# YBZh/Point-DAE

Hardware: AMD Instinct MI355X
Metric: pretrain point-clouds/sec (N=1024,G=64) (higher is better)
Workload: dtype f32 (3xbf16 exact-split operands, fp32 accumulate); 1 GPU; cfg3/cfg4: pretrain_PointCAE_transformer_dropout_patch_affine_r3_maskpatch_p0005_whole.yaml full train step (fwd+loss+bwd+AdamW); local_batch=128, global_batch=128, npoints=1024, num_group=64, group_size=32, parallelism=dp1, launch=hipGraph replay, reductions=float atomics, grad_allreduce=none (1 rank)

## Files before the change

### point_dae_amd/csrc/block.hip

```cpp
#include "common.h"

namespace pdae {

__device__ __forceinline__ float wave_sum(float v) {
#pragma unroll
  for (int o = 32; o >= 1; o >>= 1) v += __shfl_xor(v, o, kWave);
  return v;
}

constexpr int LN_MAX4 = 8;

__global__ __launch_bounds__(256) void add_layernorm_fwd_kernel(
    int M, int C, const float* __restrict__ x, const float* __restrict__ pos,
    const float* __restrict__ gamma, const float* __restrict__ beta, float eps,
    float* __restrict__ xsum, float* __restrict__ y, float* __restrict__ mean,
    float* __restrict__ rstd, const float* __restrict__ br, const float* __restrict__ bias,
    const float* __restrict__ keep, int T, int br_slabs) {
  const int row = blockIdx.x * 4 + (threadIdx.x >> 6);
  if (row >= M) return;
  const int lane = lane_id();
  const int n4 = C >> 2;
  const float k = keep ? keep[row / T] : 1.f;
  float4 v[LN_MAX4];
  float s = 0.f;
#pragma unroll
  for (int i = 0; i < LN_MAX4; ++i) {
    const int c4 = lane + i * kWave;
    if (c4 < n4) {
      float4 a = *reinterpret_cast<const float4*>(x + (size_t)row * C + c4 * 4);
      if (br) {
        float4 t = *reinterpret_cast<const float4*>(br + (size_t)row * C + c4 * 4);
        for (int q = 1; q < br_slabs; ++q) {
          const float4 u = *reinterpret_cast<const float4*>(br + ((size_t)q * M + row) * C + c4 * 4);
          t.x += u.x, t.y += u.y, t.z += u.z, t.w += u.w;
        }
        if (bias) {
          const float4 b = *reinterpret_cast<const float4*>(bias + c4 * 4);
          t.x += b.x, t.y += b.y, t.z += b.z, t.w += b.w;
        }
        if (keep) t.x *= k, t.y *= k, t.z *= k, t.w *= k;
        a.x += t.x, a.y += t.y, a.z += t.z, a.w += t.w;
      }
      if (pos) {
        const float4 p = *reinterpret_cast<const float4*>(pos + (size_t)row * C + c4 * 4);
        a.x += p.x, a.y += p.y, a.z += p.z, a.w += p.w;
      }
      if (pos || br) store_wt4(xsum + (size_t)row * C + c4 * 4, a);
      v[i] = a;
      s += (a.x + a.y) + (a.z + a.w);
    }
  }
  const float mu = wave_sum(s) / (float)C;
  float q = 0.f;
#pragma unroll
  for (int i = 0; i < LN_MAX4; ++i) {
    const int c4 = lane + i * kWave;
    if (c4 < n4) {
      const float dx = v[i].x - mu, dy = v[i].y - mu, dz = v[i].z - mu, dw = v[i].w - mu;
      q += (dx * dx + dy * dy) + (dz * dz + dw * dw);
    }
  }
  const float rs = rsqrtf(wave_sum(q) / (float)C + eps);
  if (lane == 0) {
    mean[row] = mu;
    rstd[row] = rs;
  }
#pragma unroll
  for (int i = 0; i < LN_MAX4; ++i) {
    const int c4 = lane + i * kWave;
    if (c4 < n4) {
      const float4 g = *reinterpret_cast<const float4*>(gamma + c4 * 4);
      const float4 b = *reinterpret_cast<const float4*>(beta + c4 * 4);
      float4 o;
      o.x = (v[i].x - mu) * rs * g.x + b.x;
      o.y = (v[i].y - mu) * rs * g.y + b.y;
      o.z = (v[i].z - mu) * rs * g.z + b.z;
      o.w = (v[i].w - mu) * rs * g.w + b.w;
      store_wt4(y + (size_t)row * C + c4 * 4, o);
    }
  }
}

template <int NS, int NW>
__global__ __launch_bounds__(NW * 64) void layernorm_bwd_kernel(
    int M, int C, int rows, const float* __restrict__ dy, const float* __restrict__ x,
    const float* __restrict__ mean, const float* __restrict__ rstd,
    const float* __restrict__ gamma, const float* __restrict__ dres, float* __restrict__ dx,
    float* __restrict__ dgamma, float* __restrict__ dbeta, const float* __restrict__ keep, int T,
    float* __restrict__ da, float* __restrict__ dbias, int dy_slabs, float* __restrict__ dacc, int dacc_mode,
    float* __restrict__ part) {
  extern __shared__ float red[];
  const int lane = lane_id(), w = threadIdx.x >> 6;
  const int n4 = C >> 2;
  const float4 zero4 = make_float4(0.f, 0.f, 0.f, 0.f);
  float4 ag[NS], ab[NS], g[NS], ac[NS];
#pragma unroll
  for (int i = 0; i < NS; ++i) {
    ag[i] = ab[i] = ac[i] = zero4;
    const int c4 = lane + i * kWave;
    g[i] = c4 < n4 ? *reinterpret_cast<const float4*>(gamma + c4 * 4) : zero4;
  }
  float4 d[NS], xv[NS], e[NS];
  float mu = 0.f, rs = 0.f, kp = 1.f;
  auto load_row = [&](int row) {
#pragma unroll
    for (int i = 0; i < NS; ++i) {
      const int c4 = lane + i * kWave;
      const bool on = c4 < n4 && row < M;
      const size_t off = (size_t)row * C + c4 * 4;
      d[i] = on ? *reinterpret_cast<const float4*>(dy + off) : zero4;
      for (int q = 1; q < dy_slabs; ++q) {
        const float4 u = on ? *reinterpret_cast<const float4*>(dy + (size_t)q * M * C + off) : zero4;
        d[i].x += u.x, d[i].y += u.y, d[i].z += u.z, d[i].w += u.w;
      }
      xv[i] = on ? *reinterpret_cast<const float4*>(x + off) : zero4;
      e[i] = (on && dres) ? *reinterpret_cast<const float4*>(dres + off) : zero4;
    }
    mu = row < M ? mean[row] : 0.f;
    rs = row < M ? rstd[row] : 0.f;
    kp = (keep && row < M) ? keep[row / T] : 1.f;
  };
  const int row0 = blockIdx.x * rows + w;
  load_row(row0);
  for (int rr = 0; rr < rows / NW; ++rr) {
    const int row = row0 + rr * NW;
    if (row >= M) break;
    float4 gd[NS], xh[NS];
    float s1 = 0.f, s2 = 0.f;
    const float rs_ = rs, kp_ = kp;
#pragma unroll
    for (int i = 0; i < NS; ++i) {
      xh[i] = make_float4((xv[i].x - mu) * rs, (xv[i].y - mu) * rs, (xv[i].z - mu) * rs, (xv[i].w - mu) * rs);
      gd[i] = make_float4(d[i].x * g[i].x, d[i].y * g[i].y, d[i].z * g[i].z, d[i].w * g[i].w);
      s1 += (gd[i].x + gd[i].y) + (gd[i].z + gd[i].w);
      s2 += (gd[i].x * xh[i].x + gd[i].y * xh[i].y) + (gd[i].z * xh[i].z + gd[i].w * xh[i].w);
      ag[i].x += d[i].x * xh[i].x, ag[i].y += d[i].y * xh[i].y, ag[i].z += d[i].z * xh[i].z, ag[i].w += d[i].w * xh[i].w;
      ab[i].x += d[i].x, ab[i].y += d[i].y, ab[i].z += d[i].z, ab[i].w += d[i].w;
    }
    float4 sk[NS];
#pragma unroll
    for (int i = 0; i < NS; ++i) sk[i] = e[i];
    if (rr + 1 < rows / NW) load_row(row + NW);
    const float m1 = wave_sum(s1) / (float)C, m2 = wave_sum(s2) / (float)C;
#pragma unroll
    for (int i = 0; i < NS; ++i) {
      const int c4 = lane + i * kWave;
      if (c4 < n4) {
        float4 o;
        o.x = rs_ * (gd[i].x - m1 - xh[i].x * m2) + sk[i].x;
        o.y = rs_ * (gd[i].y - m1 - xh[i].y * m2) + sk[i].y;
        o.z = rs_ * (gd[i].z - m1 - xh[i].z * m2) + sk[i].z;
        o.w = rs_ * (gd[i].w - m1 - xh[i].w * m2) + sk[i].w;
        store_wt4(dx + (size_t)row * C + c4 * 4, o);
        if (dacc_mode == 1) {
          store_wt4(dacc + (size_t)row * C + c4 * 4, o);
        } else if (dacc_mode == 2) {
          float4 t = *reinterpret_cast<const float4*>(dacc + (size_t)row * C + c4 * 4);
          t.x += o.x, t.y += o.y, t.z += o.z, t.w += o.w;
          *reinterpret_cast<float4*>(dacc + (size_t)row * C + c4 * 4) = t;
        }
        if (dbias) {
          if (keep) o.x *= kp_, o.y *= kp_, o.z *= kp_, o.w *= kp_;
          if (da) store_wt4(da + (size_t)row * C + c4 * 4, o);
          ac[i].x += o.x, ac[i].y += o.y, ac[i].z += o.z, ac[i].w += o.w;
        }
      }
    }
  }
  const int nred = dbias ? 3 : 2;
  float* mine = red + (size_t)w * nred * C;
#pragma unroll
  for (int i = 0; i < NS; ++i) {
    const int c4 = lane + i * kWave;
    if (c4 < n4) {
      *reinterpret_cast<float4*>(mine + c4 * 4) = ag[i];
      *reinterpret_cast<float4*>(mine + C + c4 * 4) = ab[i];
      if (dbias) *reinterpret_cast<float4*>(mine + 2 * C + c4 * 4) = ac[i];
    }
  }
  __syncthreads();
  for (int c = threadIdx.x; c < nred * C; c += NW * 64) {
    float t = 0.f;
#pragma unroll 4
    for (int k = 0; k < NW; ++k) t += red[(size_t)k * nred * C + c];
    col_add(c < C ? dgamma + c : (c < 2 * C ? dbeta + (c - C) : dbias + (c - 2 * C)), part, blockIdx.x,
            nred * C, c, t);
  }
}

__global__ __launch_bounds__(256) void bias_gelu_fwd_kernel(long long n4, int C4,
                                                            const float4* __restrict__ z,
                                                            const float4* __restrict__ bias,
                                                            float4* __restrict__ h) {
  const long long i = (long long)blockIdx.x * 256 + threadIdx.x;
  if (i >= n4) return;
  const float4 v = z[i], b = bias[i % C4];
  h[i] = make_float4(gelu_f(v.x + b.x), gelu_f(v.y + b.y), gelu_f(v.z + b.z), gelu_f(v.w + b.w));
}

constexpr int CS_NW = 16, CS_ROWS = 4 * CS_NW;
__device__ __forceinline__ void colsum_finish(float4 s, float4 (*part)[64], float* __restrict__ out, int c,
                                              int N, float* __restrict__ det) {
  const int lane = threadIdx.x & 63, w = threadIdx.x >> 6;
  part[w][lane] = s;
  __syncthreads();
  if (w == 0 && c < N && out) {
    float4 t = part[0][lane];
#pragma unroll
    for (int k = 1; k < CS_NW; ++k) {
      const float4 u = part[k][lane];
      t.x += u.x, t.y += u.y, t.z += u.z, t.w += u.w;
    }
    if (det) {
      *reinterpret_cast<float4*>(det + (size_t)blockIdx.y * N + c) = t;
    } else {
      atomicAdd(out + c + 0, t.x), atomicAdd(out + c + 1, t.y);
      atomicAdd(out + c + 2, t.z), atomicAdd(out + c + 3, t.w);
    }
  }
}

__global__ __launch_bounds__(CS_NW * 64) void bias_gelu_bwd_kernel(int M, int C, const float* __restrict__ z,
                                                            const float* __restrict__ bias,
                                                            const float* __restrict__ dh,
                                                            float* __restrict__ dz,
                                                            float* __restrict__ dbias,
                                                            int rows_per_split, float* __restrict__ det) {
  __shared__ float4 part[CS_NW][64];
  const int lane = threadIdx.x & 63, w = threadIdx.x >> 6;
  const int c = (blockIdx.x * 64 + lane) * 4;
  const int mbeg = blockIdx.y * rows_per_split, mend = min(M, mbeg + rows_per_split);
  float4 s = make_float4(0.f, 0.f, 0.f, 0.f);
  if (c < C) {
    const float4 b = *reinterpret_cast<const float4*>(bias + c);
#pragma unroll 4
    for (int m = mbeg + w; m < mend; m += CS_NW) {
      const float4 v = *reinterpret_cast<const float4*>(z + (size_t)m * C + c);
      const float4 d = *reinterpret_cast<const float4*>(dh + (size_t)m * C + c);
      float4 o;
      o.x = d.x * gelu_grad_f(v.x + b.x);
      o.y = d.y * gelu_grad_f(v.y + b.y);
      o.z = d.z * gelu_grad_f(v.z + b.z);
      o.w = d.w * gelu_grad_f(v.w + b.w);
      *reinterpret_cast<float4*>(dz + (size_t)m * C + c) = o;
      s.x += o.x, s.y += o.y, s.z += o.z, s.w += o.w;
    }
  }
  colsum_finish(s, part, dbias, c, C, det);
}

__global__ __launch_bounds__(256) void gelu_fwd_kernel(long long n4, const float4* __restrict__ z,
                                                       float4* __restrict__ h) {
  const long long i = (long long)blockIdx.x * 256 + threadIdx.x;
  if (i >= n4) return;
  const float4 v = z[i];
  h[i] = make_float4(gelu_f(v.x), gelu_f(v.y), gelu_f(v.z), gelu_f(v.w));
}

__global__ __launch_bounds__(256) void gelu_bwd_kernel(long long n4, const float4* __restrict__ z,
                                                       const float4* __restrict__ dh,
                                                       float4* __restrict__ dz) {
  const long long i = (long long)blockIdx.x * 256 + threadIdx.x;
  if (i >= n4) return;
  const float4 v = z[i], d = dh[i];
  dz[i] = make_float4(d.x * gelu_grad_f(v.x), d.y * gelu_grad_f(v.y), d.z * gelu_grad_f(v.z),
                      d.w * gelu_grad_f(v.w));
}

__global__ __launch_bounds__(256) void scale_residual_kernel(long long n4, int C4, int T,
                                                             const float4* __restrict__ a,
                                                             const float4* __restrict__ bias,
                                                             const float* __restrict__ keep,
                                                             const float4* __restrict__ res,
                                                             float4* __restrict__ y) {
  const long long i = (long long)blockIdx.x * 256 + threadIdx.x;
  if (i >= n4) return;
  const long long row = i / C4;
  float4 v = a[i];
  if (bias) {
    const float4 b = bias[i - row * C4];
    v.x += b.x, v.y += b.y, v.z += b.z, v.w += b.w;
  }
  if (keep) {
    const float k = keep[row / T];
    v.x *= k, v.y *= k, v.z *= k, v.w *= k;
  }
  if (res) {
    const float4 r = res[i];
    v.x += r.x, v.y += r.y, v.z += r.z, v.w += r.w;
  }
  y[i] = v;
}

template <int LPR>
__global__ __launch_bounds__(CS_NW * 64) void colsum2_kernel(int M, int N, const float* __restrict__ X,
                                                             float* __restrict__ out, int rows_per_split,
                                                             float* __restrict__ det) {
  __shared__ float4 part[CS_NW][64];
  constexpr int RPW = 64 / LPR;
  const int lane = threadIdx.x & 63, w = threadIdx.x >> 6;
  const int c = (blockIdx.x * 64 + (lane % LPR)) * 4;
  const int mbeg = blockIdx.y * rows_per_split, mend = min(M, mbeg + rows_per_split);
  float4 s = make_float4(0.f, 0.f, 0.f, 0.f);
  if (c < N) {
#pragma unroll 4
    for (int m = mbeg + w * RPW + lane / LPR; m < mend; m += CS_NW * RPW) {
      const float4 v = *reinterpret_cast<const float4*>(X + (size_t)m * N + c);
      s.x += v.x, s.y += v.y, s.z += v.z, s.w += v.w;
    }
  }
  if (LPR < 64) {
#pragma unroll
    for (int o = 32; o >= LPR; o >>= 1) {
      s.x += __shfl_xor(s.x, o, kWave), s.y += __shfl_xor(s.y, o, kWave);
      s.z += __shfl_xor(s.z, o, kWave), s.w += __shfl_xor(s.w, o, kWave);
    }
    if (lane >= LPR) s = make_float4(0.f, 0.f, 0.f, 0.f), part[w][lane] = s;
  }
  colsum_finish(s, part, (LPR < 64 && lane >= LPR) ? nullptr : out, c, N, det);
}

__global__ __launch_bounds__(CS_NW * 64) void scale_colsum_kernel(int M, int N, int T,
                                                                  const float* __restrict__ X,
                                                                  const float* __restrict__ keep,
                                                                  float* __restrict__ Y, float* __restrict__ out,
                                                                  int rows_per_split, float* __restrict__ det) {
  __shared__ float4 part[CS_NW][64];
  const int lane = threadIdx.x & 63, w = threadIdx.x >> 6;
  const int c = (blockIdx.x * 64 + lane) * 4;
  const int mbeg = blockIdx.y * rows_per_split, mend = min(M, mbeg + rows_per_split);
  float4 s = make_float4(0.f, 0.f, 0.f, 0.f);
  if (c < N) {
#pragma unroll 4
    for (int m = mbeg + w; m < mend; m += CS_NW) {
      float4 v = *reinterpret_cast<const float4*>(X + (size_t)m * N + c);
      const float k = keep[m / T];
      v.x *= k, v.y *= k, v.z *= k, v.w *= k;
      *reinterpret_cast<float4*>(Y + (size_t)m * N + c) = v;
      s.x += v.x, s.y += v.y, s.z += v.z, s.w += v.w;
    }
  }
  colsum_finish(s, part, out, c, N, det);
}

}

using namespace pdae;

static int cs_rows(int M) {
  int rows = CS_ROWS;
  if ((M + rows - 1) / rows > 256) rows = CS_NW * ((M + 256 * CS_NW - 1) / (256 * CS_NW));
  return rows;
}

static int ln_forward(const char* what, int M, int C, int T, const float* x, const float* br,
                      const float* bias, const float* keep, const float* pos, const float* gamma,
                      const float* beta, float eps, float* xsum, float* y, float* mean, float* rstd,
                      int br_slabs, pdae_stream_t stream) {
  if (M < 0 || C <= 0 || C % 4 != 0 || C > 4 * kWave * LN_MAX4 || T <= 0 || br_slabs < 1 || br_slabs > 8)
    return bad_arg("layernorm forward: C must be a multiple of 4, at most 2048; T > 0; 1..8 slabs");
  if (M == 0) return PDAE_OK;
  if (!x || !gamma || !beta || !y || !mean || !rstd || ((pos || br) && !xsum) || ((bias || keep) && !br))
    return bad_arg("layernorm forward: null pointer");
  hipLaunchKernelGGL(add_layernorm_fwd_kernel, dim3((M + 3) / 4), dim3(256), 0, as_stream(stream), M,
                     C, x, pos, gamma, beta, eps, xsum, y, mean, rstd, br, bias, keep, T, br_slabs);
  return check_launch(what);
}

extern "C" int pdae_add_layernorm_forward(int M, int C, const float* x, const float* pos,
                                          const float* gamma, const float* beta, float eps,
                                          float* xsum, float* y, float* mean, float* rstd,
                                          pdae_stream_t stream) {
  return ln_forward("add_layernorm_forward", M, C, 1, x, nullptr, nullptr, nullptr, pos, gamma, beta, eps,
                    xsum, y, mean, rstd, 1, stream);
}

extern "C" int pdae_residual_layernorm_forward(int M, int C, int T, const float* a, int a_slabs, const float* bias,
                                               const float* keep, const float* res, const float* pos,
                                               const float* gamma, const float* beta, float eps,
                                               float* xsum, float* y, float* mean, float* rstd,
                                               pdae_stream_t stream) {
  if (!a) return bad_arg("residual_layernorm_forward: null pointer");
  return ln_forward("residual_layernorm_forward", M, C, T, res, a, bias, keep, pos, gamma, beta, eps, xsum,
                    y, mean, rstd, a_slabs, stream);
}

static int ln_backward(const char* what, int M, int C, int T, const float* dy, int dy_slabs, const float* x,
                       const float* mean, const float* rstd, const float* gamma, const float* dres,
                       const float* keep, float* dx, float* da, float* dgamma, float* dbeta, float* dbias,
                       int accumulate, float* dacc, int dacc_mode, pdae_stream_t stream) {
  if (dacc_mode < 0 || dacc_mode > 2 || (dacc_mode && !dacc)) return bad_arg("layernorm backward: bad dacc");
  if (M < 0 || C <= 0 || C % 4 != 0 || C > 4 * kWave * LN_MAX4 || T <= 0 || dy_slabs < 1 || dy_slabs > 8)
    return bad_arg("layernorm backward: C must be a multiple of 4, at most 2048; T > 0; 1..8 slabs");
  if (!dgamma || !dbeta) return bad_arg("layernorm backward: null pointer");
  hipStream_t s = as_stream(stream);
  if (!accumulate) {
    (void)hipMemsetAsync(dgamma, 0, sizeof(float) * C, s);
    (void)hipMemsetAsync(dbeta, 0, sizeof(float) * C, s);
    if (dbias) (void)hipMemsetAsync(dbias, 0, sizeof(float) * C, s);
  }
  if (M == 0) return check_launch(what);
  if (!dy || !x || !mean || !rstd || !gamma || !dx || ((keep || da) && !dbias) || (keep && !da))
    return bad_arg("layernorm backward: null pointer");
  const int nred = dbias ? 3 : 2;
  int rows, blocks;
  if (C <= 512) {
    rows = 16 * (M >= 6144 ? 2 : 1);
  } else {
    rows = 4 * ((M + 4 * 256 - 1) / (4 * 256));
    if (rows > 32) rows = 32;
  }
  blocks = (M + rows - 1) / rows;
  int rc = PDAE_OK;
  float* part = static_cast<float*>(det_workspace(sizeof(float) * (size_t)blocks * nred * C, &rc));
  if (rc) return rc;
  bool parked = false;
  if (!part && (part = deferred_take(blocks, nred * C, dgamma, C, dbeta, C, dbias, dbias ? C : 0))) parked = true;
  if (C <= 512)
    hipLaunchKernelGGL((layernorm_bwd_kernel<2, 16>), dim3(blocks), dim3(1024), 16 * nred * C * sizeof(float), s, M,
                       C, rows, dy, x, mean, rstd, gamma, dres, dx, dgamma, dbeta, keep, T, da, dbias, dy_slabs,
                       dacc, dacc_mode, part);
  else
    hipLaunchKernelGGL((layernorm_bwd_kernel<LN_MAX4, 4>), dim3(blocks), dim3(256), 4 * nred * C * sizeof(float), s,
                       M, C, rows, dy, x, mean, rstd, gamma, dres, dx, dgamma, dbeta, keep, T, da, dbias, dy_slabs,
                       dacc, dacc_mode, part);
  if (part && !parked) return det_reduce(s, blocks, nred * C, part, dgamma, C, dbeta, C, dbias, dbias ? C : 0);
  return check_launch(what);
}

extern "C" int pdae_layernorm_backward(int M, int C, const float* dy, int dy_slabs, const float* x,
                                       const float* mean, const float* rstd, const float* gamma,
                                       const float* dres, float* dx, float* dgamma, float* dbeta,
                                       int accumulate, float* dacc, int dacc_mode, pdae_stream_t stream) {
  return ln_backward("layernorm_backward", M, C, 1, dy, dy_slabs, x, mean, rstd, gamma, dres, nullptr, dx, nullptr,
                     dgamma, dbeta, nullptr, accumulate, dacc, dacc_mode, stream);
}

extern "C" int pdae_residual_layernorm_backward(int M, int C, int T, const float* dy, int dy_slabs, const float* x,
                                                const float* mean, const float* rstd,
                                                const float* gamma, const float* dres,
                                                const float* keep, float* dx, float* da, float* dgamma,
                                                float* dbeta, float* dbias, int accumulate,
                                                float* dacc, int dacc_mode, pdae_stream_t stream) {
  if (!dbias) return bad_arg("residual_layernorm_backward: null pointer");
  return ln_backward("residual_layernorm_backward", M, C, T, dy, dy_slabs, x, mean, rstd, gamma, dres, keep, dx, da,
                     dgamma, dbeta, dbias, accumulate, dacc, dacc_mode, stream);
}

extern "C" int pdae_gelu_forward(long long n, const float* z, float* h, pdae_stream_t stream) {
  if (n < 0 || n % 4 != 0) return bad_arg("gelu_forward: n must be a multiple of 4");
  if (n == 0) return PDAE_OK;
  if (!z || !h) return bad_arg("gelu_forward: null pointer");
  hipLaunchKernelGGL(gelu_fwd_kernel, dim3((unsigned)((n / 4 + 255) / 256)), dim3(256), 0,
                     as_stream(stream), n / 4, reinterpret_cast<const float4*>(z),
                     reinterpret_cast<float4*>(h));
  return check_launch("gelu_forward");
}

extern "C" int pdae_gelu_backward(long long n, const float* z, const float* dh, float* dz,
                                  pdae_stream_t stream) {
  if (n < 0 || n % 4 != 0) return bad_arg("gelu_backward: n must be a multiple of 4");
  if (n == 0) return PDAE_OK;
  if (!z || !dh || !dz) return bad_arg("gelu_backward: null pointer");
  hipLaunchKernelGGL(gelu_bwd_kernel, dim3((unsigned)((n / 4 + 255) / 256)), dim3(256), 0,
                     as_stream(stream), n / 4, reinterpret_cast<const float4*>(z),
                     reinterpret_cast<const float4*>(dh), reinterpret_cast<float4*>(dz));
  return check_launch("gelu_backward");
}

extern "C" int pdae_bias_gelu_forward(int M, int C, const float* z, const float* bias, float* h,
                                      pdae_stream_t stream) {
  if (M < 0 || C <= 0 || C % 4 != 0) return bad_arg("bias_gelu_forward: C must be a positive multiple of 4");
  if (M == 0) return PDAE_OK;
  if (!z || !bias || !h) return bad_arg("bias_gelu_forward: null pointer");
  const long long n4 = (long long)M * (C / 4);
  hipLaunchKernelGGL(bias_gelu_fwd_kernel, dim3((unsigned)((n4 + 255) / 256)), dim3(256), 0,
                     as_stream(stream), n4, C / 4, reinterpret_cast<const float4*>(z),
                     reinterpret_cast<const float4*>(bias), reinterpret_cast<float4*>(h));
  return check_launch("bias_gelu_forward");
}

extern "C" int pdae_bias_gelu_backward(int M, int C, const float* z, const float* bias,
                                       const float* dh, float* dz, float* dbias, int accumulate,
                                       pdae_stream_t stream) {
  if (M < 0 || C <= 0 || C % 4 != 0) return bad_arg("bias_gelu_backward: C must be a positive multiple of 4");
  if (!dbias) return bad_arg("bias_gelu_backward: null pointer");
  hipStream_t s = as_stream(stream);
  if (!accumulate) (void)hipMemsetAsync(dbias, 0, sizeof(float) * (size_t)C, s);
  if (M == 0) return check_launch("bias_gelu_backward");
  if (!z || !bias || !dh || !dz) return bad_arg("bias_gelu_backward: null pointer");
  const int rows = cs_rows(M), P = (M + rows - 1) / rows;
  int rc = PDAE_OK;
  float* det = static_cast<float*>(det_workspace(sizeof(float) * (size_t)P * C, &rc));
  if (rc) return rc;
  hipLaunchKernelGGL(bias_gelu_bwd_kernel, dim3((C + 255) / 256, P), dim3(CS_NW * 64), 0, s, M, C, z, bias, dh, dz,
                     dbias, rows, det);
  if (det) return det_reduce(s, P, C, det, dbias, C);
  return check_launch("bias_gelu_backward");
}

extern "C" int pdae_scale_residual(int M, int C, int T, const float* a, const float* bias,
                                   const float* keep, const float* res, float* y,
                                   pdae_stream_t stream) {
  if (M < 0 || C <= 0 || C % 4 != 0 || T <= 0) return bad_arg("scale_residual: bad size");
  if (M == 0) return PDAE_OK;
  if (!a || !y) return bad_arg("scale_residual: null pointer");
  const long long n4 = (long long)M * (C / 4);
  hipLaunchKernelGGL(scale_residual_kernel, dim3((unsigned)((n4 + 255) / 256)), dim3(256), 0,
                     as_stream(stream), n4, C / 4, T, reinterpret_cast<const float4*>(a),
                     reinterpret_cast<const float4*>(bias), keep, reinterpret_cast<const float4*>(res),
                     reinterpret_cast<float4*>(y));
  return check_launch("scale_residual");
}

extern "C" int pdae_colsum(int M, int N, const float* X, float* out, int accumulate,
                           pdae_stream_t stream) {
  if (M < 0 || N <= 0 || N % 4 != 0) return bad_arg("colsum: N must be a positive multiple of 4");
  if (!out) return bad_arg("colsum: null pointer");
  hipStream_t s = as_stream(stream);
  if (!accumulate) (void)hipMemsetAsync(out, 0, sizeof(float) * (size_t)N, s);
  if (M == 0) return check_launch("colsum");
  if (!X) return bad_arg("colsum: null pointer");
  const int rows = cs_rows(M), P = (M + rows - 1) / rows;
  int rc = PDAE_OK;
  float* det = static_cast<float*>(det_workspace(sizeof(float) * (size_t)P * N, &rc));
  if (rc) return rc;
  if (N == 128)
    hipLaunchKernelGGL(colsum2_kernel<32>, dim3(1, P), dim3(CS_NW * 64), 0, s, M, N, X, out, rows, det);
  else if (N == 64)
    hipLaunchKernelGGL(colsum2_kernel<16>, dim3(1, P), dim3(CS_NW * 64), 0, s, M, N, X, out, rows, det);
  else
    hipLaunchKernelGGL(colsum2_kernel<64>, dim3((N + 255) / 256, P), dim3(CS_NW * 64), 0, s, M, N, X, out, rows, det);
  if (det) return det_reduce(s, P, N, det, out, N);
  return check_launch("colsum");
}

extern "C" int pdae_scale_colsum(int M, int N, int T, const float* X, const float* keep, float* Y,
                                 float* out, int accumulate, pdae_stream_t stream) {
  if (M < 0 || N <= 0 || N % 4 != 0 || T <= 0) return bad_arg("scale_colsum: N must be a positive multiple of 4, T > 0");
  hipStream_t s = as_stream(stream);
  if (out && !accumulate) (void)hipMemsetAsync(out, 0, sizeof(float) * (size_t)N, s);
  if (M == 0) return check_launch("scale_colsum");
  if (!X || !keep || !Y) return bad_arg("scale_colsum: null pointer");
  const int rows = cs_rows(M), P = (M + rows - 1) / rows;
  int rc = PDAE_OK;
  float* det = out ? static_cast<float*>(det_workspace(sizeof(float) * (size_t)P * N, &rc)) : nullptr;
  if (rc) return rc;
  hipLaunchKernelGGL(scale_colsum_kernel, dim3((N + 255) / 256, P), dim3(CS_NW * 64), 0, s, M, N, T, X, keep, Y,
                     out, rows, det);
  if (det) return det_reduce(s, P, N, det, out, N);
  return check_launch("scale_colsum");
}


namespace pdae {

__global__ __launch_bounds__(256) void drop_path_keep_kernel(int n, int B, const float* __restrict__ r,
                                                             const float* __restrict__ keep, float* __restrict__ out) {
  const int i = blockIdx.x * 256 + threadIdx.x;
  if (i >= n) return;
  const float k = keep[i / B];
  out[i] = floorf(r[i] + k) / k;
}

__global__ __launch_bounds__(256) void pos_embed_fc1_kernel(int M, int H, const float* __restrict__ xyz,
                                                            const long long* __restrict__ rows,
                                                            const float* __restrict__ w1, const float* __restrict__ b1,
                                                            float* __restrict__ h, float* __restrict__ gp,
                                                            float* __restrict__ xp) {
  const int q = H / 4;
  const long long i = (long long)blockIdx.x * 256 + threadIdx.x;
  if (i >= (long long)M * q) return;
  const int m = (int)(i / q), c = (int)(i % q) * 4;
  const long long src = rows ? rows[m] : m;
  const float x0 = xyz[src * 3 + 0], x1 = xyz[src * 3 + 1], x2 = xyz[src * 3 + 2];
  if (c == 0) *reinterpret_cast<float4*>(xp + (size_t)m * 4) = make_float4(x0, x1, x2, 0.f);
  float hv[4], gv[4];
#pragma unroll
  for (int e = 0; e < 4; ++e) {
    const float* w = w1 + (size_t)(c + e) * 3;
    const float z = fmaf(x2, w[2], fmaf(x1, w[1], x0 * w[0])) + b1[c + e];
    const float cdf = 0.5f * (1.0f + erff(z * 0.70710678118654752440f));
    const float pdf = 0.39894228040143267794f * expf(-0.5f * z * z);
    hv[e] = z * cdf, gv[e] = cdf + z * pdf;
  }
  *reinterpret_cast<float4*>(h + (size_t)m * H + c) = make_float4(hv[0], hv[1], hv[2], hv[3]);
  *reinterpret_cast<float4*>(gp + (size_t)m * H + c) = make_float4(gv[0], gv[1], gv[2], gv[3]);
}

__global__ __launch_bounds__(256) void tail_rows_gather_kernel(long long n4, int C4, int T, int tail, const float4* __restrict__ a,
                                                               const float4* __restrict__ b, float4* __restrict__ a_t,
                                                               float4* __restrict__ b_t) {
  const long long i = (long long)blockIdx.x * 256 + threadIdx.x;
  if (i >= n4) return;
  const long long row = i / C4;
  const int c = (int)(i - row * C4);
  const long long smp = row / tail;
  const long long src = (smp * T + (T - tail) + (row - smp * tail)) * C4 + c;
  a_t[i] = a[src];
  if (b) b_t[i] = b[src];
}
__global__ __launch_bounds__(256) void tail_rows_scatter_kernel(long long n4, int C4, int T, int tail, const float4* __restrict__ da_t,
                                                                const float4* __restrict__ db_t, float4* __restrict__ da,
                                                                float4* __restrict__ db) {
  const long long i = (long long)blockIdx.x * 256 + threadIdx.x;
  if (i >= n4) return;
  const long long row = i / C4;
  const int c = (int)(i - row * C4);
  const long long smp = row / T;
  const int t = (int)(row - smp * T) - (T - tail);
  const float4 zero = make_float4(0.f, 0.f, 0.f, 0.f);
  const long long src = (smp * tail + t) * C4 + c;
  da[i] = t >= 0 ? da_t[src] : zero;
  if (db) db[i] = t >= 0 ? db_t[src] : zero;
}

__global__ __launch_bounds__(256) void slab_sum_epi_kernel(long long n4, int N4, int S, const float4* __restrict__ slabs,
                                                           const float4* __restrict__ bias, int epi,
                                                           const float4* __restrict__ z, float4* __restrict__ y) {
  const long long i = (long long)blockIdx.x * 256 + threadIdx.x;
  if (i >= n4) return;
  float4 a = slabs[i];
  for (int q = 1; q < S; ++q) {
    const float4 v = slabs[(size_t)q * n4 + i];
    a.x += v.x, a.y += v.y, a.z += v.z, a.w += v.w;
  }
  if (bias) {
    const float4 b = bias[i % N4];
    a.x += b.x, a.y += b.y, a.z += b.z, a.w += b.w;
  }
  if (epi == 1) a.x = a.x > 0.f ? a.x : 0.f, a.y = a.y > 0.f ? a.y : 0.f, a.z = a.z > 0.f ? a.z : 0.f, a.w = a.w > 0.f ? a.w : 0.f;
  if (epi == 4) {
    const float4 m = z[i];
    a.x = m.x > 0.f ? a.x : 0.f, a.y = m.y > 0.f ? a.y : 0.f, a.z = m.z > 0.f ? a.z : 0.f, a.w = m.w > 0.f ? a.w : 0.f;
  }
  y[i] = a;
}

}

static int tail_check(int B, int T, int tail, int C) {
  if (B < 0 || T <= 0 || tail <= 0 || tail > T || C <= 0 || C % 4 != 0) return bad_arg("tail_rows: B >= 0, 0 < tail <= T, C a positive multiple of 4");
  return PDAE_OK;
}
extern "C" int pdae_tail_rows_gather(int B, int T, int tail, int C, const float* a, const float* b, float* a_t, float* b_t,
                                     pdae_stream_t stream) {
  using namespace pdae;
  int rc = tail_check(B, T, tail, C);
  if (rc) return rc;
  if (B == 0) return PDAE_OK;
  if (!a || !a_t || (b && !b_t)) return bad_arg("tail_rows_gather: null pointer");
  const long long n4 = (long long)B * tail * (C / 4);
  hipLaunchKernelGGL(tail_rows_gather_kernel, dim3((unsigned)((n4 + 255) / 256)), dim3(256), 0, as_stream(stream), n4, C / 4, T, tail,
                     reinterpret_cast<const float4*>(a), reinterpret_cast<const float4*>(b), reinterpret_cast<float4*>(a_t),
                     reinterpret_cast<float4*>(b_t));
  return check_launch("tail_rows_gather");
}
extern "C" int pdae_tail_rows_scatter(int B, int T, int tail, int C, const float* da_t, const float* db_t, float* da, float* db,
                                      pdae_stream_t stream) {
  using namespace pdae;
  int rc = tail_check(B, T, tail, C);
  if (rc) return rc;
  if (B == 0) return PDAE_OK;
  if (!da_t || !da || (db && !db_t)) return bad_arg("tail_rows_scatter: null pointer");
  const long long n4 = (long long)B * T * (C / 4);
  hipLaunchKernelGGL(tail_rows_scatter_kernel, dim3((unsigned)((n4 + 255) / 256)), dim3(256), 0, as_stream(stream), n4, C / 4, T, tail,
                     reinterpret_cast<const float4*>(da_t), reinterpret_cast<const float4*>(db_t), reinterpret_cast<float4*>(da),
                     reinterpret_cast<float4*>(db));
  return check_launch("tail_rows_scatter");
}

extern "C" int pdae_slab_sum_epi(int S, int M, int N, const float* slabs, const float* bias, int epi, const float* Z, float* Y,
                                 pdae_stream_t stream) {
  using namespace pdae;
  if (S <= 0 || S > 8 || M < 0 || N <= 0 || N % 4 != 0) return bad_arg("slab_sum_epi: 1..8 slabs, M >= 0, N a positive multiple of 4");
  if (epi != 0 && epi != 1 && epi != 4) return bad_arg("slab_sum_epi: epi 0 (store), 1 (ReLU) or 4 (mask by Z > 0)");
  if (M == 0) return PDAE_OK;
  if (!slabs || !Y || (epi == 4 && !Z)) return bad_arg("slab_sum_epi: null pointer");
  const long long n4 = (long long)M * (N / 4);
  hipLaunchKernelGGL(slab_sum_epi_kernel, dim3((unsigned)((n4 + 255) / 256)), dim3(256), 0, as_stream(stream), n4, N / 4, S,
                     reinterpret_cast<const float4*>(slabs), reinterpret_cast<const float4*>(bias), epi,
                     reinterpret_cast<const float4*>(Z), reinterpret_cast<float4*>(Y));
  return check_launch("slab_sum_epi");
}

extern "C" int pdae_drop_path_keep(int sites, int B, const float* r, const float* keep, float* out, pdae_stream_t stream) {
  using namespace pdae;
  if (sites < 0 || B < 0) return bad_arg("drop_path_keep: negative size");
  if (sites == 0 || B == 0) return PDAE_OK;
  if (!r || !keep || !out) return bad_arg("drop_path_keep: null pointer");
  const int n = sites * B;
  hipLaunchKernelGGL(drop_path_keep_kernel, dim3((n + 255) / 256), dim3(256), 0, as_stream(stream), n, B, r, keep, out);
  return check_launch("drop_path_keep");
}

extern "C" int pdae_pos_embed_fc1(int M, int H, const float* xyz, const int64_t* rows, const float* w1, const float* b1,
                                  float* h, float* gp, float* xp, pdae_stream_t stream) {
  using namespace pdae;
  if (M < 0 || H <= 0 || H % 4 != 0) return bad_arg("pos_embed_fc1: M >= 0, H a positive multiple of 4 required");
  if (M == 0) return PDAE_OK;
  if (!xyz || !w1 || !b1 || !h || !gp || !xp) return bad_arg("pos_embed_fc1: null pointer");
  const long long n = (long long)M * (H / 4);
  hipLaunchKernelGGL(pos_embed_fc1_kernel, dim3((unsigned)((n + 255) / 256)), dim3(256), 0, as_stream(stream), M, H, xyz,
                     reinterpret_cast<const long long*>(rows), w1, b1, h, gp, xp);
  return check_launch("pos_embed_fc1");
}
```

Before: 13230 clouds/s.

## Specialize layernorm kernels by slab count, bias, pos and residual flags

Adds templated forward and backward layernorm kernels, specialized at compile time on column-chunk count, number of summed slabs and whether bias, pos or residual inputs exist. The forward kernel issues all loads up front, and the backward kernel prefetches the next row and the dacc value ahead of the reduction, so memory latency overlaps with compute. The tail scatter kernel now skips its loads for padded rows. An environment variable can fall back to the legacy kernels, and the extra instantiations cost code size and register pressure.

```diff
diff --git a/point_dae_amd/csrc/block.hip b/point_dae_amd/csrc/block.hip
--- a/point_dae_amd/csrc/block.hip
+++ b/point_dae_amd/csrc/block.hip
@@ -1,3 +1,6 @@
+#include <stdlib.h>
+#include <string.h>
+
 #include "common.h"
 
 namespace pdae {
@@ -10,7 +13,7 @@
 
 constexpr int LN_MAX4 = 8;
 
-__global__ __launch_bounds__(256) void add_layernorm_fwd_kernel(
+__global__ __launch_bounds__(256) void add_layernorm_fwd_legacy_kernel(
     int M, int C, const float* __restrict__ x, const float* __restrict__ pos,
     const float* __restrict__ gamma, const float* __restrict__ beta, float eps,
     float* __restrict__ xsum, float* __restrict__ y, float* __restrict__ mean,
@@ -81,8 +84,99 @@
   }
 }
 
+__device__ __forceinline__ float4 ld4(const float* p) { return *reinterpret_cast<const float4*>(p); }
+__device__ __forceinline__ void add4(float4& a, const float4& b) { a.x += b.x, a.y += b.y, a.z += b.z, a.w += b.w; }
+
+template <int NS, int SLABS, bool BIAS, bool POS>
+__global__ __launch_bounds__(256) void add_layernorm_fwd_kernel(
+    int M, int C, const float* __restrict__ x, const float* __restrict__ pos,
+    const float* __restrict__ gamma, const float* __restrict__ beta, float eps,
+    float* __restrict__ xsum, float* __restrict__ y, float* __restrict__ mean,
+    float* __restrict__ rstd, const float* __restrict__ br, const float* __restrict__ bias,
+    const float* __restrict__ keep, int T, int br_slabs) {
+  constexpr bool BR = SLABS != 0;
+  constexpr int SL = SLABS > 0 ? SLABS : 1;
+  const int row = blockIdx.x * 4 + (threadIdx.x >> 6);
+  if (row >= M) return;
+  const int lane = lane_id();
+  const int n4 = C >> 2;
+  const float4 zero4 = make_float4(0.f, 0.f, 0.f, 0.f);
+  float k = 1.f;
+  if (keep) k = keep[row / T];
+  float4 v[NS], u[SL][NS], bb[NS], pp[NS], g[NS], be[NS];
+#pragma unroll
+  for (int i = 0; i < NS; ++i) {
+    v[i] = bb[i] = pp[i] = g[i] = be[i] = zero4;
+#pragma unroll
+    for (int q = 0; q < SL; ++q) u[q][i] = zero4;
+    const int c4 = lane + i * kWave;
+    if (c4 < n4) {
+      const size_t off = (size_t)row * C + c4 * 4;
+      v[i] = ld4(x + off);
+      if (BR) {
+#pragma unroll
+        for (int q = 0; q < SL; ++q) u[q][i] = ld4(br + (size_t)q * M * C + off);
+      }
+      if (POS) pp[i] = ld4(pos + off);
+      if (BR && BIAS) bb[i] = ld4(bias + c4 * 4);
+      g[i] = ld4(gamma + c4 * 4);
+      be[i] = ld4(beta + c4 * 4);
+    }
+  }
+  float s = 0.f;
+#pragma unroll
+  for (int i = 0; i < NS; ++i) {
+    const int c4 = lane + i * kWave;
+    if (c4 < n4) {
+      float4 a = v[i];
+      if (BR) {
+        float4 t = u[0][i];
+#pragma unroll
+        for (int q = 1; q < SL; ++q) add4(t, u[q][i]);
+        if (SLABS < 0) {
+          for (int q = 1; q < br_slabs; ++q) add4(t, ld4(br + ((size_t)q * M + row) * C + c4 * 4));
+        }
+        if (BIAS) add4(t, bb[i]);
+        if (keep) t.x *= k, t.y *= k, t.z *= k, t.w *= k;
+        add4(a, t);
+      }
+      if (POS) add4(a, pp[i]);
+      if (POS || BR) store_wt4(xsum + (size_t)row * C + c4 * 4, a);
+      v[i] = a;
+      s += (a.x + a.y) + (a.z + a.w);
+    }
+  }
+  const float mu = wave_sum(s) / (float)C;
+  float q = 0.f;
+#pragma unroll
+  for (int i = 0; i < NS; ++i) {
+    const int c4 = lane + i * kWave;
+    if (c4 < n4) {
+      const float dx = v[i].x - mu, dy = v[i].y - mu, dz = v[i].z - mu, dw = v[i].w - mu;
+      q += (dx * dx + dy * dy) + (dz * dz + dw * dw);
+    }
+  }
+  const float rs = rsqrtf(wave_sum(q) / (float)C + eps);
+  if (lane == 0) {
+    mean[row] = mu;
+    rstd[row] = rs;
+  }
+#pragma unroll
+  for (int i = 0; i < NS; ++i) {
+    const int c4 = lane + i * kWave;
+    if (c4 < n4) {
+      float4 o;
+      o.x = (v[i].x - mu) * rs * g[i].x + be[i].x;
+      o.y = (v[i].y - mu) * rs * g[i].y + be[i].y;
+      o.z = (v[i].z - mu) * rs * g[i].z + be[i].z;
+      o.w = (v[i].w - mu) * rs * g[i].w + be[i].w;
+      store_wt4(y + (size_t)row * C + c4 * 4, o);
+    }
+  }
+}
+
 template <int NS, int NW>
-__global__ __launch_bounds__(NW * 64) void layernorm_bwd_kernel(
+__global__ __launch_bounds__(NW * 64) void layernorm_bwd_legacy_kernel(
     int M, int C, int rows, const float* __restrict__ dy, const float* __restrict__ x,
     const float* __restrict__ mean, const float* __restrict__ rstd,
     const float* __restrict__ gamma, const float* __restrict__ dres, float* __restrict__ dx,
@@ -157,6 +251,135 @@
         } else if (dacc_mode == 2) {
           float4 t = *reinterpret_cast<const float4*>(dacc + (size_t)row * C + c4 * 4);
           t.x += o.x, t.y += o.y, t.z += o.z, t.w += o.w;
+          *reinterpret_cast<float4*>(dacc + (size_t)row * C + c4 * 4) = t;
+        }
+        if (dbias) {
+          if (keep) o.x *= kp_, o.y *= kp_, o.z *= kp_, o.w *= kp_;
+          if (da) store_wt4(da + (size_t)row * C + c4 * 4, o);
+          ac[i].x += o.x, ac[i].y += o.y, ac[i].z += o.z, ac[i].w += o.w;
+        }
+      }
+    }
+  }
+  const int nred = dbias ? 3 : 2;
+  float* mine = red + (size_t)w * nred * C;
+#pragma unroll
+  for (int i = 0; i < NS; ++i) {
+    const int c4 = lane + i * kWave;
+    if (c4 < n4) {
+      *reinterpret_cast<float4*>(mine + c4 * 4) = ag[i];
+      *reinterpret_cast<float4*>(mine + C + c4 * 4) = ab[i];
+      if (dbias) *reinterpret_cast<float4*>(mine + 2 * C + c4 * 4) = ac[i];
+    }
+  }
+  __syncthreads();
+  for (int c = threadIdx.x; c < nred * C; c += NW * 64) {
+    float t = 0.f;
+#pragma unroll 4
+    for (int k = 0; k < NW; ++k) t += red[(size_t)k * nred * C + c];
+    col_add(c < C ? dgamma + c : (c < 2 * C ? dbeta + (c - C) : dbias + (c - 2 * C)), part, blockIdx.x,
+            nred * C, c, t);
+  }
+}
+
+template <int NS, int NW, int SLABS, int RPW, bool DRES>
+__global__ __launch_bounds__(NW * 64) void layernorm_bwd_kernel(
+    int M, int C, int rows, const float* __restrict__ dy, const float* __restrict__ x,
+    const float* __restrict__ mean, const float* __restrict__ rstd,
+    const float* __restrict__ gamma, const float* __restrict__ dres, float* __restrict__ dx,
+    float* __restrict__ dgamma, float* __restrict__ dbeta, const float* __restrict__ keep, int T,
+    float* __restrict__ da, float* __restrict__ dbias, int dy_slabs, float* __restrict__ dacc, int dacc_mode,
+    float* __restrict__ part) {
+  constexpr int SL = SLABS > 0 ? SLABS : 1;
+  extern __shared__ float red[];
+  const int lane = lane_id(), w = threadIdx.x >> 6;
+  const int n4 = C >> 2;
+  const float4 zero4 = make_float4(0.f, 0.f, 0.f, 0.f);
+  float4 ag[NS], ab[NS], g[NS], ac[NS];
+#pragma unroll
+  for (int i = 0; i < NS; ++i) {
+    ag[i] = ab[i] = ac[i] = g[i] = zero4;
+    const int c4 = lane + i * kWave;
+    if (c4 < n4) g[i] = ld4(gamma + c4 * 4);
+  }
+  float4 u[SL][NS], xv[NS], e[NS];
+  float mu = 0.f, rs = 0.f, kp = 1.f;
+  auto issue = [&](int row) {
+    mu = 0.f, rs = 0.f, kp = 1.f;
+#pragma unroll
+    for (int i = 0; i < NS; ++i) {
+      xv[i] = e[i] = zero4;
+#pragma unroll
+      for (int q = 0; q < SL; ++q) u[q][i] = zero4;
+    }
+    if (row < M) {
+#pragma unroll
+      for (int i = 0; i < NS; ++i) {
+        const int c4 = lane + i * kWave;
+        if (c4 < n4) {
+          const size_t off = (size_t)row * C + c4 * 4;
+#pragma unroll
+          for (int q = 0; q < SL; ++q) u[q][i] = ld4(dy + (size_t)q * M * C + off);
+          xv[i] = ld4(x + off);
+          if (DRES) e[i] = ld4(dres + off);
+        }
+      }
+      mu = mean[row];
+      rs = rstd[row];
+      if (keep) kp = keep[row / T];
+    }
+  };
+  const int row0 = blockIdx.x * rows + w;
+  const int nrr = RPW ? RPW : rows / NW;
+  issue(row0);
+  for (int rr = 0; rr < nrr; ++rr) {
+    const int row = row0 + rr * NW;
+    if (row >= M) break;
+    float4 old[NS];
+#pragma unroll
+    for (int i = 0; i < NS; ++i) {
+      old[i] = zero4;
+      const int c4 = lane + i * kWave;
+      if (dacc_mode == 2 && c4 < n4) old[i] = ld4(dacc + (size_t)row * C + c4 * 4);
+    }
+    float4 gd[NS], xh[NS], sk[NS];
+    float s1 = 0.f, s2 = 0.f;
+    const float rs_ = rs, kp_ = kp;
+#pragma unroll
+    for (int i = 0; i < NS; ++i) {
+      float4 d = u[0][i];
+#pragma unroll
+      for (int q = 1; q < SL; ++q) add4(d, u[q][i]);
+      if (SLABS < 0) {
+        const int c4 = lane + i * kWave;
+        if (c4 < n4)
+          for (int q = 1; q < dy_slabs; ++q) add4(d, ld4(dy + ((size_t)q * M + row) * C + c4 * 4));
+      }
+      xh[i] = make_float4((xv[i].x - mu) * rs, (xv[i].y - mu) * rs, (xv[i].z - mu) * rs, (xv[i].w - mu) * rs);
+      gd[i] = make_float4(d.x * g[i].x, d.y * g[i].y, d.z * g[i].z, d.w * g[i].w);
+      s1 += (gd[i].x + gd[i].y) + (gd[i].z + gd[i].w);
+      s2 += (gd[i].x * xh[i].x + gd[i].y * xh[i].y) + (gd[i].z * xh[i].z + gd[i].w * xh[i].w);
+      ag[i].x += d.x * xh[i].x, ag[i].y += d.y * xh[i].y, ag[i].z += d.z * xh[i].z, ag[i].w += d.w * xh[i].w;
+      ab[i].x += d.x, ab[i].y += d.y, ab[i].z += d.z, ab[i].w += d.w;
+      sk[i] = e[i];
+    }
+    if (RPW != 1 && rr + 1 < nrr) issue(row + NW);
+    const float m1 = wave_sum(s1) / (float)C, m2 = wave_sum(s2) / (float)C;
+#pragma unroll
+    for (int i = 0; i < NS; ++i) {
+      const int c4 = lane + i * kWave;
+      if (c4 < n4) {
+        float4 o;
+        o.x = rs_ * (gd[i].x - m1 - xh[i].x * m2) + sk[i].x;
+        o.y = rs_ * (gd[i].y - m1 - xh[i].y * m2) + sk[i].y;
+        o.z = rs_ * (gd[i].z - m1 - xh[i].z * m2) + sk[i].z;
+        o.w = rs_ * (gd[i].w - m1 - xh[i].w * m2) + sk[i].w;
+        store_wt4(dx + (size_t)row * C + c4 * 4, o);
+        if (dacc_mode == 1) {
+          store_wt4(dacc + (size_t)row * C + c4 * 4, o);
+        } else if (dacc_mode == 2) {
+          float4 t = old[i];
+          add4(t, o);
           *reinterpret_cast<float4*>(dacc + (size_t)row * C + c4 * 4) = t;
         }
         if (dbias) {
@@ -353,6 +576,70 @@
   return rows;
 }
 
+static int ln_form() {
+  static const int form = [] {
+    const char* e = getenv("PDAE_LN");
+    if (!e || !e[0] || e[0] == '1') return 7;
+    if (e[0] == '0') return 0;
+    return (strchr(e, 'f') ? 1 : 0) | (strchr(e, 'b') ? 2 : 0) | (strchr(e, 't') ? 4 : 0);
+  }();
+  return form;
+}
+
+template <int NS, int SLABS, typename... Args>
+static void ln_fwd_launch2(bool has_bias, bool has_pos, int M, hipStream_t s, Args... args) {
+  const dim3 grid((M + 3) / 4), block(256);
+  if (SLABS != 0 && has_bias) {
+    if (has_pos) hipLaunchKernelGGL((add_layernorm_fwd_kernel<NS, SLABS, SLABS != 0, true>), grid, block, 0, s, M, args...);
+    else hipLaunchKernelGGL((add_layernorm_fwd_kernel<NS, SLABS, SLABS != 0, false>), grid, block, 0, s, M, args...);
+  } else {
+    if (has_pos) hipLaunchKernelGGL((add_layernorm_fwd_kernel<NS, SLABS, false, true>), grid, block, 0, s, M, args...);
+    else hipLaunchKernelGGL((add_layernorm_fwd_kernel<NS, SLABS, false, false>), grid, block, 0, s, M, args...);
+  }
+}
+
+template <int NS>
+static void ln_fwd_launch(int slabs, int M, int C, const float* x, const float* pos, const float* gamma,
+                          const float* beta, float eps, float* xsum, float* y, float* mean, float* rstd,
+                          const float* br, const float* bias, const float* keep, int T, int br_slabs, hipStream_t s) {
+#define PDAE_LN_FWD(SL)                                                                                             \
+  ln_fwd_launch2<NS, SL>(bias != nullptr, pos != nullptr, M, s, C, x, pos, gamma, beta, eps, xsum, y, mean, rstd, \
+                         br, bias, keep, T, br_slabs)
+  switch (slabs) {
+    case 0: PDAE_LN_FWD(0); break;
+    case 1: PDAE_LN_FWD(1); break;
+    case 2: PDAE_LN_FWD(2); break;
+    case 3: if constexpr (NS == 2) { PDAE_LN_FWD(3); break; }
+    case 4: if constexpr (NS == 2) { PDAE_LN_FWD(4); break; }
+    default: PDAE_LN_FWD(-1); break;
+  }
+#undef PDAE_LN_FWD
+}
+
+template <int NS, int NW, int RPW>
+static void ln_bwd_launch(int slabs, int blocks, size_t lds, hipStream_t s, int M, int C, int rows, const float* dy,
+                          const float* x, const float* mean, const float* rstd, const float* gamma,
+                          const float* dres, float* dx, float* dgamma, float* dbeta, const float* keep, int T,
+                          float* da, float* dbias, int dy_slabs, float* dacc, int dacc_mode, float* part) {
+#define PDAE_LN_BWD2(SL, DR)                                                                                        \
+  hipLaunchKernelGGL((layernorm_bwd_kernel<NS, NW, SL, RPW, DR>), dim3(blocks), dim3(NW * 64), lds, s, M, C, rows, dy, \
+                     x, mean, rstd, gamma, dres, dx, dgamma, dbeta, keep, T, da, dbias, dy_slabs, dacc, dacc_mode, part)
+#define PDAE_LN_BWD(SL)         \
+  do {                          \
+    if (dres) PDAE_LN_BWD2(SL, true);  \
+    else PDAE_LN_BWD2(SL, false);      \
+  } while (0)
+  switch (slabs) {
+    case 1: PDAE_LN_BWD(1); break;
+    case 2: PDAE_LN_BWD(2); break;
+    case 3: if constexpr (NS == 2) { PDAE_LN_BWD(3); break; }
+    case 4: if constexpr (NS == 2 && RPW == 1) { PDAE_LN_BWD(4); break; }
+    default: PDAE_LN_BWD(-1); break;
+  }
+#undef PDAE_LN_BWD
+#undef PDAE_LN_BWD2
+}
+
 static int ln_forward(const char* what, int M, int C, int T, const float* x, const float* br,
                       const float* bias, const float* keep, const float* pos, const float* gamma,
                       const float* beta, float eps, float* xsum, float* y, float* mean, float* rstd,
@@ -362,8 +649,18 @@
   if (M == 0) return PDAE_OK;
   if (!x || !gamma || !beta || !y || !mean || !rstd || ((pos || br) && !xsum) || ((bias || keep) && !br))
     return bad_arg("layernorm forward: null pointer");
-  hipLaunchKernelGGL(add_layernorm_fwd_kernel, dim3((M + 3) / 4), dim3(256), 0, as_stream(stream), M,
-                     C, x, pos, gamma, beta, eps, xsum, y, mean, rstd, br, bias, keep, T, br_slabs);
+  if (!(ln_form() & 1)) {
+    hipLaunchKernelGGL(add_layernorm_fwd_legacy_kernel, dim3((M + 3) / 4), dim3(256), 0, as_stream(stream), M,
+                       C, x, pos, gamma, beta, eps, xsum, y, mean, rstd, br, bias, keep, T, br_slabs);
+    return check_launch(what);
+  }
+  const int slabs = !br ? 0 : (br_slabs <= (C <= 512 ? 4 : 2) ? br_slabs : -1);
+  if (C <= 512)
+    ln_fwd_launch<2>(slabs, M, C, x, pos, gamma, beta, eps, xsum, y, mean, rstd, br, bias, keep, T, br_slabs,
+                     as_stream(stream));
+  else
+    ln_fwd_launch<LN_MAX4>(slabs, M, C, x, pos, gamma, beta, eps, xsum, y, mean, rstd, br, bias, keep, T, br_slabs,
+                           as_stream(stream));
   return check_launch(what);
 }
 
@@ -416,14 +713,26 @@
   if (rc) return rc;
   bool parked = false;
   if (!part && (part = deferred_take(blocks, nred * C, dgamma, C, dbeta, C, dbias, dbias ? C : 0))) parked = true;
-  if (C <= 512)
-    hipLaunchKernelGGL((layernorm_bwd_kernel<2, 16>), dim3(blocks), dim3(1024), 16 * nred * C * sizeof(float), s, M,
-                       C, rows, dy, x, mean, rstd, gamma, dres, dx, dgamma, dbeta, keep, T, da, dbias, dy_slabs,
-                       dacc, dacc_mode, part);
-  else
-    hipLaunchKernelGGL((layernorm_bwd_kernel<LN_MAX4, 4>), dim3(blocks), dim3(256), 4 * nred * C * sizeof(float), s,
-                       M, C, rows, dy, x, mean, rstd, gamma, dres, dx, dgamma, dbeta, keep, T, da, dbias, dy_slabs,
-                       dacc, dacc_mode, part);
+  const int slabs = dy_slabs <= (C > 512 ? 2 : (rows == 16 ? 4 : 3)) ? dy_slabs : -1;
+  if (!(ln_form() & 2)) {
+    if (C <= 512)
+      hipLaunchKernelGGL((layernorm_bwd_legacy_kernel<2, 16>), dim3(blocks), dim3(1024), 16 * nred * C * sizeof(float),
+                         s, M, C, rows, dy, x, mean, rstd, gamma, dres, dx, dgamma, dbeta, keep, T, da, dbias,
+                         dy_slabs, dacc, dacc_mode, part);
+    else
+      hipLaunchKernelGGL((layernorm_bwd_legacy_kernel<LN_MAX4, 4>), dim3(blocks), dim3(256),
+                         4 * nred * C * sizeof(float), s, M, C, rows, dy, x, mean, rstd, gamma, dres, dx, dgamma,
+                         dbeta, keep, T, da, dbias, dy_slabs, dacc, dacc_mode, part);
+  } else if (C <= 512 && rows == 16) {
+    ln_bwd_launch<2, 16, 1>(slabs, blocks, 16 * nred * C * sizeof(float), s, M, C, rows, dy, x, mean, rstd, gamma,
+                            dres, dx, dgamma, dbeta, keep, T, da, dbias, dy_slabs, dacc, dacc_mode, part);
+  } else if (C <= 512) {
+    ln_bwd_launch<2, 16, 2>(slabs, blocks, 16 * nred * C * sizeof(float), s, M, C, rows, dy, x, mean, rstd, gamma,
+                            dres, dx, dgamma, dbeta, keep, T, da, dbias, dy_slabs, dacc, dacc_mode, part);
+  } else {
+    ln_bwd_launch<LN_MAX4, 4, 0>(slabs, blocks, 4 * nred * C * sizeof(float), s, M, C, rows, dy, x, mean, rstd, gamma,
+                                 dres, dx, dgamma, dbeta, keep, T, da, dbias, dy_slabs, dacc, dacc_mode, part);
+  }
   if (part && !parked) return det_reduce(s, blocks, nred * C, part, dgamma, C, dbeta, C, dbias, dbias ? C : 0);
   return check_launch(what);
 }
@@ -600,7 +909,7 @@
   a_t[i] = a[src];
   if (b) b_t[i] = b[src];
 }
-__global__ __launch_bounds__(256) void tail_rows_scatter_kernel(long long n4, int C4, int T, int tail, const float4* __restrict__ da_t,
+__global__ __launch_bounds__(256) void tail_rows_scatter_legacy_kernel(long long n4, int C4, int T, int tail, const float4* __restrict__ da_t,
                                                                 const float4* __restrict__ db_t, float4* __restrict__ da,
                                                                 float4* __restrict__ db) {
   const long long i = (long long)blockIdx.x * 256 + threadIdx.x;
@@ -614,6 +923,24 @@
   da[i] = t >= 0 ? da_t[src] : zero;
   if (db) db[i] = t >= 0 ? db_t[src] : zero;
 }
+__global__ __launch_bounds__(256) void tail_rows_scatter_kernel(long long n4, int C4, int T, int tail, const float4* __restrict__ da_t,
+                                                                const float4* __restrict__ db_t, float4* __restrict__ da,
+                                                                float4* __restrict__ db) {
+  const long long i = (long long)blockIdx.x * 256 + threadIdx.x;
+  if (i >= n4) return;
+  const long long row = i / C4;
+  const int c = (int)(i - row * C4);
+  const long long smp = row / T;
+  const int t = (int)(row - smp * T) - (T - tail);
+  const long long src = (smp * tail + t) * C4 + c;
+  float4 va = make_float4(0.f, 0.f, 0.f, 0.f), vb = va;
+  if (t >= 0) {
+    va = da_t[src];
+    if (db) vb = db_t[src];
+  }
+  da[i] = va;
+  if (db) db[i] = vb;
+}
 
 __global__ __launch_bounds__(256) void slab_sum_epi_kernel(long long n4, int N4, int S, const float4* __restrict__ slabs,
                                                            const float4* __restrict__ bias, int epi,
@@ -664,9 +991,9 @@
   if (B == 0) return PDAE_OK;
   if (!da_t || !da || (db && !db_t)) return bad_arg("tail_rows_scatter: null pointer");
   const long long n4 = (long long)B * T * (C / 4);
-  hipLaunchKernelGGL(tail_rows_scatter_kernel, dim3((unsigned)((n4 + 255) / 256)), dim3(256), 0, as_stream(stream), n4, C / 4, T, tail,
-                     reinterpret_cast<const float4*>(da_t), reinterpret_cast<const float4*>(db_t), reinterpret_cast<float4*>(da),
-                     reinterpret_cast<float4*>(db));
+  hipLaunchKernelGGL((ln_form() & 4) ? tail_rows_scatter_kernel : tail_rows_scatter_legacy_kernel, dim3((unsigned)((n4 + 255) / 256)),
+                     dim3(256), 0, as_stream(stream), n4, C / 4, T, tail, reinterpret_cast<const float4*>(da_t),
+                     reinterpret_cast<const float4*>(db_t), reinterpret_cast<float4*>(da), reinterpret_cast<float4*>(db));
   return check_launch("tail_rows_scatter");
 }
 
```

New measurement: 13520 clouds/s, median of 6. +2.2%, better.
